# RMichelsen/VulkanHybridRenderer

Hardware: AMD Instinct MI355X
Metric: Mrays/s (unique rays) + ms/frame, Sponza 1080p RT shadows+AO+SVGF (higher is better)
Workload: dtype f32

## Files before the change

### vulkanhybridrenderer_amd/csrc/kernels_trace.hip

```cpp
#define VHR_TRACE_UNIT unit_trace
#include <cstring>

#include "trace_queue.hpp"
#include "svgf_temporal.hpp"

namespace vhr {

#ifndef VHR_REDO_INLINE
#define VHR_REDO_INLINE __attribute__((noinline))
#endif
#ifndef VHR_K1_WAVES_MIN
#define VHR_K1_WAVES_MIN 8
#endif
constexpr uint32_t kRedoPixel = 0x80000000u;

struct RaygenArgs {
    DeviceScene scene;
    vhr_per_frame_data pfd;
    vhr_trace_params tp;
    const void *normals;
    const float *depth;
    void *shadow_ao;
    void *reflections;
    uint32_t width, height;
// ... 20 lines not shown
    N = f3{ nid.x, nid.y, nid.z };
    origin = P + N * a.tp.normal_bias;
    Hit hit;

    float rnd1 = random01(rng);
    float rnd2 = random01(rng);
    shadow_payload = 1.0f;
    if (a.tp.shadow_enable) {
        const f3 cone_dir = normalize3(uniform_sample_cone(rnd1, rnd2, a.tp.cone_cos_max));
        const f3 dir = onb_transform(L, cone_dir);
        const bool occluded = traverse<true, STRIDE>(a.scene, origin, dir, a.tp.tmin, a.tp.tmax, stack, hit, overflow, ray_filter<FILTER>(a.scene, a.masks, a.masks.shadow));
        shadow_payload = occluded ? 0.0f : 1.0f;
    }
    ao_payload = 0.0f;
    for (uint32_t i = 0; i < a.tp.ao_spp; ++i) {
        rnd1 = random01(rng);
        rnd2 = random01(rng);
        const f3 rnd_dir = cosine_hemisphere(rnd1, rnd2);
        const f3 dir = onb_transform(N, rnd_dir);
        const bool occluded = traverse<true, STRIDE>(a.scene, origin, dir, a.tp.tmin, a.tp.ao_tmax, stack, hit, overflow, ray_filter<FILTER>(a.scene, a.masks, a.masks.ao));
        ao_payload += occluded ? 0.0f : 1.0f;
    }
    if (a.tp.ao_spp) ao_payload /= float(a.tp.ao_spp); else ao_payload = 1.0f;
}

template <int FILTER = kFilterNone>
__device__ VHR_REDO_INLINE float2 redo_pixel_visibility(const RaygenArgs *a, const uint32_t x, const uint32_t y) {
    int st[kTraceStack];
    uint32_t overflow = 0;
    f3 P, N, origin;
    float shadow_payload, ao_payload;
    pixel_visibility<1, FILTER>(*a, x, y, a->depth[size_t(y) * a->width + x], st, overflow, P, N, origin, shadow_payload, ao_payload);
    return float2{ shadow_payload, ao_payload };
}

template <int FILTER = kFilterNone>
__device__ __forceinline__ void raygen_pixel(const RaygenArgs &a, const uint32_t x, const uint32_t y, int *stack, uint32_t &overflow, bool &covered, bool &second_ray) {
    const uint32_t W = a.width;
    const float depth = a.depth[size_t(y) * W + x];
    if (depth == 0.0f) {
        store_rg16f(a.shadow_ao, W, x, y, 1.0f, 1.0f);
        if (a.reflections) store_rgba16f(a.reflections, W, x, y, 0.0f, 0.0f, 0.0f, 0.0f);
        return;
    }
    covered = true;
    f3 P, N, origin;
    float shadow_payload, ao_payload;
    pixel_visibility<kTraceBlock, FILTER>(a, x, y, depth, stack, overflow, P, N, origin, shadow_payload, ao_payload);
    store_rg16f(a.shadow_ao, W, x, y, shadow_payload, ao_payload);

    if (a.reflections) {
        f4 payload = f4{ 0.0f, 0.0f, 0.0f, 0.0f };
        if (a.tp.reflections) {
            const f3 cam = f3{ a.pfd.camera_view_inverse[12], a.pfd.camera_view_inverse[13], a.pfd.camera_view_inverse[14] };
            const f3 I = normalize3(P - cam);
            const float ni2 = 2.0f * dot3(N, I);
            const f3 rdir = I - N * ni2;
            payload = trace_reflection<kTraceBlock>(a.scene, a.pfd, a.tp, origin, rdir, stack, overflow, second_ray, ray_filter<FILTER>(a.scene, a.masks, a.masks.reflection));
        }
        store_rgba16f(a.reflections, W, x, y, payload.x, payload.y, payload.z, payload.w);
    }
}

template <int FILTER = kFilterNone>
__global__ __launch_bounds__(kTraceBlock) void raygen_kernel(const RaygenArgs a, const Stamps st) {
    vhr_stamp(st);
    __shared__ int s_stack[kTraceStack * kTraceBlock];
    int *stack = s_stack + threadIdx.x;
    uint32_t x, y;
    pixel_of_thread(x, y, a.row_begin);
    uint32_t overflow = 0;
    bool covered = false, second_ray = false;
    if (x < a.width && y < a.row_end) raygen_pixel<FILTER>(a, x, y, stack, overflow, covered, second_ray);
    if (a.stats) {
        const unsigned long long cov = __ballot(covered), ovf = __ballot(overflow != 0), sec = __ballot(second_ray);
        if ((threadIdx.x & 63u) == 0) {
            if (cov) atomicAdd(&a.stats->covered_pixels, (unsigned long long)__popcll(cov));
            if (ovf) atomicAdd(&a.stats->stack_overflows, (unsigned long long)__popcll(ovf));
            if (sec) atomicAdd(&a.stats->second_bounce_rays, (unsigned long long)__popcll(sec));
        }
    }
}

template <int WAVES, bool COMPACT, bool SPILL, bool STATS, bool FUSE = false, int FILTER = kFilterNone>
__global__ __launch_bounds__(kQueueBlock *WAVES) __attribute__((amdgpu_waves_per_eu(VHR_K1_WAVES_MIN, 8))) void raygen_queue_kernel(const RaygenArgs a, const uint32_t stack_levels, const uint32_t refill_threshold,
                                                                          const uint32_t block_tiles_x, const uint32_t early_exit, const uint32_t tile_rows, const uint32_t steal_threshold, const Stamps st) {
    vhr_stamp(st);
    RayStats *const stats = STATS ? a.stats : nullptr;
    extern __shared__ int s_dyn[];
    const unsigned long long t_start = stats ? __builtin_readcyclecounter() : 0ull;
    unsigned long long t_setup = 0, t_refill = 0, t_nodes = 0, t_leaves = 0, n_refills = 0;
    __shared__ uint32_t s_vis_all[WAVES][kQueueBlock];
    __shared__ float s_ray_all[WAVES][5][kQueueBlock];
    __shared__ uint8_t s_list_all[WAVES][kQueueBlock];
    __shared__ float4 s_cut_all[WAVES][kCutMax][2];
    const uint32_t lane = threadIdx.x & 63u, wave = uint32_t(__builtin_amdgcn_readfirstlane(int(threadIdx.x >> 6)));
    uint32_t (&s_vis)[kQueueBlock] = s_vis_all[wave];
    float (&s_ray)[5][kQueueBlock] = s_ray_all[wave];
    uint8_t (&s_list)[kQueueBlock] = s_list_all[wave];
    float4 (&s_cut)[kCutMax][2] = s_cut_all[wave];
    const unsigned long long t_cost0 = a.co.wave_cost ? __builtin_readcyclecounter() : 0ull;
    if constexpr (!STATS) {
        if (a.co.order_out && blockIdx.x == 0u) order_blocks_by_cost<WAVES>(a.co.cost_prev, a.co.order_blocks, a.co.order_out, reinterpret_cast<uint32_t *>(s_dyn));
    }
    int *stack = s_dyn + wave * (stack_levels + 3u) * kQueueBlock + lane;
    stack[0] = kStackSentinel;
    const uint32_t W = a.width, H = a.height;
    uint32_t x, y;
    const uint32_t block_tile = a.co.block_order ? a.co.block_order[blockIdx.x] : blockIdx.x;
    tile_pixel<WAVES>(block_tile, block_tiles_x, wave, lane, a.row_begin, tile_rows, x, y, a.col_begin);
    const bool in_range = x < a.col_end && y < a.row_end && (lane >> 3) < tile_rows;
    bool covered = false;
    float depth = 0.0f;
    if (in_range) {
        depth = a.depth[size_t(y) * W + x];
        covered = depth != 0.0f;
        if (!covered) store_rg16f(a.shadow_ao, W, x, y, 1.0f, 1.0f);
    }
    s_vis[lane] = 0;
    const uint32_t first_kind = a.tp.shadow_enable ? 0u : 1u;
    const uint32_t last_kind = a.tp.ao_spp;
    const bool ao_only = first_kind != 0u;
    const bool kind_bits = last_kind <= 30u;
    const f3 L = -f3{ a.pfd.directional_light.direction[0], a.pfd.directional_light.direction[1], a.pfd.directional_light.direction[2] };
    f3 omin = f3{ 3.0e38f, 3.0e38f, 3.0e38f }, omax = f3{ -3.0e38f, -3.0e38f, -3.0e38f };
    float ao_reach = 0.0f;
    if (covered) {
        const float u = (float(x) + 0.5f) / float(W);
        const float v = (float(y) + 0.5f) / float(H);
        const f3 P = get_world_space_position(a.pfd, depth, u, v);
        const uint2 nraw = reinterpret_cast<const uint2 *>(a.normals)[size_t(y) * W + x];
        const f3 N = f3{ half_bits_to_float(uint16_t(nraw.x & 0xffffu)), half_bits_to_float(uint16_t(nraw.x >> 16)), half_bits_to_float(uint16_t(nraw.y & 0xffffu)) };
        const f3 origin = P + N * a.tp.normal_bias;
        s_ray[0][lane] = origin.x; s_ray[1][lane] = origin.y; s_ray[2][lane] = origin.z;
        s_ray[3][lane] = __uint_as_float(nraw.x); s_ray[4][lane] = __uint_as_float(nraw.y);
        if (ao_only) ao_reach = a.tp.ao_tmax * onb_norm_bound(N);
        omin = origin; omax = origin;
    }
    const unsigned long long cov_mask = __ballot(covered);
    const uint32_t ncov = uint32_t(__popcll(cov_mask));
    if (covered) s_list[lane_rank(cov_mask)] = uint8_t(lane);
    wave_lds_sync();
    const uint32_t total = (a.scene.node_count == 0) ? 0u : ncov * (1u + last_kind - first_kind);
    uint32_t cut_n = 0;
    if (total) cut_n = build_tile_cut(a.scene, omin, omax, s_cut, lane, ao_only ? ao_reach : 3.0e38f, kCutMax, COMPACT ? int(sizeof(BvhNode16)) : int(sizeof(BvhNode48)),
                                      COMPACT ? f3{ a.scene.centre[0], a.scene.centre[1], a.scene.centre[2] } : f3{ 0.0f, 0.0f, 0.0f });
    const uint32_t n_cut_entries = cut_n;
    uint32_t emask = 0;
    if (stats) t_setup = __builtin_readcyclecounter() - t_start;

    f3 ro = f3{ 0, 0, 0 }, rd = f3{ 0, 0, 1 }, rinv = f3{ 0, 0, 0 }, noi = f3{ 0, 0, 0 }, ainv = f3{ 0, 0, 0 };
    float tmax = 0.0f;
    int cur = 0, sp = 0;
    int sbase = 0;
    uint32_t pix = 0, kind = 0;
    bool has = false;
    uint32_t next = 0;
    uint32_t overflow = 0;
    uint32_t n_nodes = 0, n_leaves = 0, n_tris = 0, n_wave_trips = 0, n_drain_trips = 0;
    uint32_t n_drain_le4 = 0, n_drain_le8 = 0, n_drain_le16 = 0;
    int spill[SPILL ? kSpillStack : 1];
    const float tmin = a.tp.tmin;
    float tmin_v = tmin;
    asm volatile("" : "+v"(tmin_v));
    for (;;) {
        const unsigned long long idle = __ballot(!has);
        const uint32_t n_idle = uint32_t(__popcll(idle));
        const unsigned long long t0 = stats ? __builtin_readcyclecounter() : 0ull;
        const bool queue_dry = next >= total;
        if (next < total && (n_idle >= refill_threshold || n_idle == 64u)) {
            __builtin_amdgcn_s_setprio(0);
            ++n_refills;
            const uint32_t r = next + lane_rank(idle);
            next += n_idle;
            if (!has && r < total) {
                uint32_t k = 0, rr = r;
                while (rr >= ncov) { rr -= ncov; ++k; }
                kind = last_kind - k;
                pix = s_list[rr];
                ro = f3{ s_ray[0][pix], s_ray[1][pix], s_ray[2][pix] };
                const uint32_t nxy = __float_as_uint(s_ray[3][pix]), nzw = __float_as_uint(s_ray[4][pix]);
                const uint32_t px = x - (lane & 7u) + (pix & 7u), py = y - (lane >> 3) + (pix >> 3);
                rd = ray_direction(a.tp, seed_thread((py * H + px) * a.pfd.frame_index), kind, L,
                                   f3{ half_bits_to_float(uint16_t(nxy & 0xffffu)), half_bits_to_float(uint16_t(nxy >> 16)), half_bits_to_float(uint16_t(nzw & 0xffffu)) });
                tmax = kind == 0 ? a.tp.tmax : a.tp.ao_tmax;
                f3 bo, bd;
                box_ray(a.scene, ro, rd, bo, bd);
                rinv = f3{ cull_reciprocal(bd.x), cull_reciprocal(bd.y), cull_reciprocal(bd.z) };
                const f3 oc = COMPACT ? f3{ bo.x - a.scene.centre[0], bo.y - a.scene.centre[1], bo.z - a.scene.centre[2] } : bo;
                noi = f3{ -(oc.x * rinv.x), -(oc.y * rinv.y), -(oc.z * rinv.z) };
                if (!COMPACT) ainv = f3{ fabsf(rinv.x), fabsf(rinv.y), fabsf(rinv.z) };
                sbase = 0;
                cut_to_stack(s_cut, cut_n, stack, stack_levels, rinv, noi, tmin_v, tmax, cur, sp, emask);
// ... 88 lines not shown
            const bool holder = has && cur < 0 && cur != kStackSentinel;
            uint32_t w = mine, hl = holder ? tot - mine : 0u, fr = holder ? 0u : tot - mine;
            for (int off = 32; off > 0; off >>= 1) { w += uint32_t(__shfl_xor(int(w), off)); hl += uint32_t(__shfl_xor(int(hl), off)); fr += uint32_t(__shfl_xor(int(fr), off)); }
            n_drain_le4 += w; n_drain_le8 += hl; n_drain_le16 += fr;
        }
#endif
        const unsigned long long t2 = stats ? __builtin_readcyclecounter() : 0ull;
        auto test_leaf = [&](const int code) {
            const uint32_t vv = ~uint32_t(code);
            const uint32_t first = vv >> 2, count = (vv & 3u) + 1u;
            ++n_leaves;
            const BvhTri *const leaf = a.scene.tris + first;
            for (uint32_t i = 0; i < count; ++i) {
                ++n_tris;
                const float4 ta = reinterpret_cast<const float4 *>(leaf + i)[0], tb = reinterpret_cast<const float4 *>(leaf + i)[1];
                const float tcx = reinterpret_cast<const float *>(leaf + i)[8];
                const f3 v0 = f3{ ta.x, ta.y, ta.z }, e1 = f3{ ta.w, tb.x, tb.y }, e2 = f3{ tb.z, tb.w, tcx };
                float ct, cu, cv;
                if (mt_candidate(ro, rd, v0, e1, e2, tmin, tmax, ct, cu, cv)) {
                    if (solution_consistent(ro, rd, v0, e1, e2, ct, cu, cv)) {
                        if constexpr (FILTER == kFilterAlpha) { if (gbuf_discarded(a.scene, first + i, cu, cv)) continue; }
                        if constexpr (FILTER == kFilterMask) {
                            if ((uint32_t(a.masks.prim_masks[leaf[i].prim]) & (kind == 0 ? a.masks.shadow : a.masks.ao)) == 0u) continue;
                            if (a.masks.alpha && gbuf_discarded(a.scene, first + i, cu, cv)) continue;
                        }
                        found = true;
                        break;
                    }
                    atomicOr(&s_vis[pix], kRedoPixel);
                }
            }
        };
        if (has && cur < 0 && cur != kStackSentinel) {
            test_leaf(cur);
            if (!found) {
                cur = stack[min(uint32_t(sp), stack_levels + 1u) * kQueueBlock];
                if (SPILL && __any(uint32_t(sp) > stack_levels)) {
                    if (uint32_t(sp) > stack_levels) cur = spill[(uint32_t(sp) - 1u - stack_levels) & uint32_t(kSpillStack - 1)];
                }
                --sp;
            }
        }
        if (has && !found && cur == kStackSentinel && emask) {
            const int e = __ffs(int(emask)) - 1;
            emask &= emask - 1u;
            cur = __float_as_int(s_cut[e][1].z);
            sp = 0;
            sbase = 0;
        }
        const bool finished = found || cur == kStackSentinel;
        if (has && finished) {
            has = false;
            if (kind_bits) { if (found) atomicOr(&s_vis[pix], 1u << kind); }
            else if (kind == 0) { if (found) atomicOr(&s_vis[pix], 1u); }
            else if (!found) atomicAdd(&s_vis[pix], 256u);
        }
        if (stats) {
            const unsigned long long t3 = __builtin_readcyclecounter();
            t_refill += t1 - t0; t_nodes += t2 - t1; t_leaves += t3 - t2;
            uint32_t tn = n_nodes - nodes_before, tt = n_tris - tris_before;
            for (int off = 32; off > 0; off >>= 1) { tn = max(tn, uint32_t(__shfl_xor(int(tn), off))); tt = max(tt, uint32_t(__shfl_xor(int(tt), off))); }
            n_wave_trips += tn + tt;
            if (next >= total) {
#ifndef VHR_K1_COUNT_TRIPS
                n_drain_trips += tn + tt;
#endif
                const uint32_t live = uint32_t(__popcll(__ballot(has)));
#ifndef VHR_K1_COUNT_IDLE
                if (live <= 4u) n_drain_le4 += tn + tt;
                if (live <= 8u) n_drain_le8 += tn + tt;
                if (live <= 16u) n_drain_le16 += tn + tt;
#endif
            }
        }
    }
    wave_lds_sync();
    float shadow_payload = 1.0f, ao_payload = 1.0f;
    uint32_t n_redo = 0;
    if (covered) {
        const uint32_t vis = s_vis[lane];
        shadow_payload = (vis & 1u) ? 0.0f : 1.0f;
        if (a.tp.ao_spp) ao_payload = float(a.scene.node_count == 0 ? a.tp.ao_spp : (kind_bits ? a.tp.ao_spp - uint32_t(__popc(vis >> 1)) : (vis >> 8))) / float(a.tp.ao_spp);
        if (vis & kRedoPixel) {
            static_assert(offsetof(RaygenArgs, scene) == 0, "the launch's arguments start with `a`");
            const float2 again = redo_pixel_visibility<FILTER>(reinterpret_cast<const RaygenArgs *>((const void *)__builtin_amdgcn_kernarg_segment_ptr()), x, y);
            shadow_payload = again.x; ao_payload = again.y;
            n_redo = 1;
        }
        store_rg16f(a.shadow_ao, W, x, y, shadow_payload, ao_payload);
    }
    if (a.co.wave_cost && lane == 0) a.co.wave_cost[block_tile * uint32_t(WAVES) + wave] = uint32_t(min(__builtin_readcyclecounter() - t_cost0, 0xffffffffull));
    if constexpr (FUSE) {
        if (a.fuse_temporal) {
            const TemporalArgs &t = a.temporal;
            if (in_range && x >= t.col_begin && x < t.limit_x && y >= t.row_begin && y < t.row_end && y < t.limit_y) {
                const uint2 nraw = reinterpret_cast<const uint2 *>(a.normals)[size_t(y) * W + x];
                const float2 cur = unpack_rg16f(pack_rg16f(shadow_payload, ao_payload));
                svgf_temporal_pixel(t, x, y, unpack_rgba16f(nraw), cur.x, cur.y);
            }
        }
    }
    if (stats) {
        const unsigned long long ovf = __ballot(overflow != 0);
        if (lane == 0) {
            if (cov_mask) atomicAdd(&stats->covered_pixels, (unsigned long long)__popcll(cov_mask));
            if (ovf) atomicAdd(&stats->stack_overflows, (unsigned long long)__popcll(ovf));
            atomicAdd(&stats->wave_iterations, (unsigned long long)n_wave_trips);
            atomicAdd(&stats->drain_iterations, (unsigned long long)n_drain_trips);
            atomicAdd(&stats->drain_le4, (unsigned long long)n_drain_le4);
            atomicAdd(&stats->drain_le8, (unsigned long long)n_drain_le8);
            atomicAdd(&stats->drain_le16, (unsigned long long)n_drain_le16);
            atomicAdd(&stats->cycles_total, __builtin_readcyclecounter() - t_start);
            atomicAdd(&stats->cycles_setup, t_setup);
            atomicAdd(&stats->cycles_refill, t_refill);
            atomicAdd(&stats->cycles_nodes, t_nodes);
            atomicAdd(&stats->cycles_leaves, t_leaves);
            atomicAdd(&stats->refills, n_refills);
            atomicAdd(&stats->waves, 1ull);
            atomicAdd(&stats->cut_entries, (unsigned long long)n_cut_entries);
        }
        const unsigned long long redo = __ballot(n_redo != 0);
        if (redo && lane == 0) atomicAdd(&stats->pending_rays, (unsigned long long)__popcll(redo));
        for (int off = 32; off > 0; off >>= 1) { n_nodes += uint32_t(__shfl_xor(int(n_nodes), off)); n_leaves += uint32_t(__shfl_xor(int(n_leaves), off)); n_tris += uint32_t(__shfl_xor(int(n_tris), off)); }
        if (lane == 0) {
            atomicAdd(&stats->node_visits, (unsigned long long)n_nodes);
            atomicAdd(&stats->leaf_visits, (unsigned long long)n_leaves);
            atomicAdd(&stats->triangle_tests, (unsigned long long)n_tris);
        }
    }
}

template <int STRIDE, int FILTER = kFilterNone>
__device__ __forceinline__ f4 reflection_payload(const RaygenArgs &a, const uint32_t x, const uint32_t y, int *stack, bool &second_ray) {
    const uint32_t W = a.width, H = a.height;
    f4 payload = f4{ 0.0f, 0.0f, 0.0f, 0.0f };
    const float depth = a.depth[size_t(y) * W + x];
    if (depth != 0.0f && a.tp.reflections) {
        const float u = (float(x) + 0.5f) / float(W), v = (float(y) + 0.5f) / float(H);
        const f3 P = get_world_space_position(a.pfd, depth, u, v);
        const f4 nid = load_rgba16f(a.normals, W, x, y);
        const f3 N = f3{ nid.x, nid.y, nid.z };
        const f3 origin = P + N * a.tp.normal_bias;
        const f3 cam = f3{ a.pfd.camera_view_inverse[12], a.pfd.camera_view_inverse[13], a.pfd.camera_view_inverse[14] };
        const f3 I = normalize3(P - cam);
        const float ni2 = 2.0f * dot3(N, I);
        const f3 rdir = I - N * ni2;
        uint32_t overflow = 0;
        payload = trace_reflection<STRIDE>(a.scene, a.pfd, a.tp, origin, rdir, stack, overflow, second_ray, ray_filter<FILTER>(a.scene, a.masks, a.masks.reflection));
    }
    return payload;
}
template <int FILTER = kFilterNone>
__device__ __forceinline__ void reflection_pixel(const RaygenArgs &a, const uint32_t x, const uint32_t y, int *stack, bool &second_ray) {
    const f4 payload = reflection_payload<kTraceBlock, FILTER>(a, x, y, stack, second_ray);
    store_rgba16f(a.reflections, a.width, x, y, payload.x, payload.y, payload.z, payload.w);
}

struct RedoReflection { f4 payload; uint32_t second; };
template <int FILTER = kFilterNone>
__device__ __attribute__((noinline)) RedoReflection redo_pixel_reflection(const RaygenArgs *a, const uint32_t x, const uint32_t y) {
    int st[kTraceStack];
    bool second_ray = false;
    const f4 payload = reflection_payload<1, FILTER>(*a, x, y, st, second_ray);
    return RedoReflection{ payload, second_ray ? 1u : 0u };
}

template <int FILTER = kFilterNone>
__global__ __launch_bounds__(kTraceBlock) void reflection_kernel(const RaygenArgs a, const Stamps st) {
    vhr_stamp(st);
    __shared__ int s_refl_stack[kTraceStack * kTraceBlock];
    int *stack = s_refl_stack + threadIdx.x;
    uint32_t x, y;
    pixel_of_thread(x, y, a.row_begin);
    bool second_ray = false;
    if (x < a.width && y < a.row_end) reflection_pixel<FILTER>(a, x, y, stack, second_ray);
    if (a.stats) {
        const unsigned long long sec = __ballot(second_ray);
        if ((threadIdx.x & 63u) == 0 && sec) atomicAdd(&a.stats->second_bounce_rays, (unsigned long long)__popcll(sec));
    }
}

__device__ __forceinline__ void mirror_ray_of_pixel(const RaygenArgs &a, f3 cam, uint32_t x, uint32_t y, float depth, f3 &origin, f3 &rdir) {
    const uint32_t W = a.width, H = a.height;
    const float u = (float(x) + 0.5f) / float(W), v = (float(y) + 0.5f) / float(H);
    const f3 P = get_world_space_position(a.pfd, depth, u, v);
    const f4 nid = load_rgba16f(a.normals, W, x, y);
    const f3 N = f3{ nid.x, nid.y, nid.z };
    origin = P + N * a.tp.normal_bias;
    const f3 I = normalize3(P - cam);
    const float ni2 = 2.0f * dot3(N, I);
    rdir = I - N * ni2;
}

template <bool SPILL, int BOUNCES, bool STATS = false, int FILTER = kFilterNone>
__global__ __launch_bounds__(kQueueBlock * 2) __attribute__((amdgpu_waves_per_eu(7, 7))) void reflection_queue_kernel(
    const RaygenArgs a, const uint32_t stack_levels, const uint32_t refill_threshold, const uint32_t tiles_x, const uint32_t tiles_total,
    const uint32_t early_exit, const Stamps st) {
    vhr_stamp(st);
    extern __shared__ int s_dyn[];
    constexpr int ROWS = BOUNCES > 1 ? 9 : 6;
    constexpr uint32_t SUBS = 1u;
    constexpr int RAYS = 64 * int(SUBS);
    __shared__ float s_ray_all[2][ROWS][RAYS];
    __shared__ uint8_t s_list_all[2][RAYS];
    __shared__ float4 s_cut_all[2][kCutMax][2];
    __shared__ uint32_t s_redo_all[2][RAYS / 32];
    const uint32_t lane = threadIdx.x & 63u, wave = uint32_t(__builtin_amdgcn_readfirstlane(int(threadIdx.x >> 6)));
    const unsigned long long t_cost0 = a.co.wave_cost ? __builtin_readcyclecounter() : 0ull;
    if (a.co.order_out && blockIdx.x == 0u) order_blocks_by_cost<2>(a.co.cost_prev, a.co.order_blocks, a.co.order_out, reinterpret_cast<uint32_t *>(s_dyn));
    const uint32_t block = a.co.block_order ? a.co.block_order[blockIdx.x] : blockIdx.x;
    const uint32_t tile = block * 2u + wave;
// ... 107 lines not shown
            static_assert(offsetof(RaygenArgs, scene) == 0, "the launch's arguments start with `a`");
            const RedoReflection again = redo_pixel_reflection<FILTER>(reinterpret_cast<const RaygenArgs *>((const void *)__builtin_amdgcn_kernarg_segment_ptr()), x, y);
            payload = again.payload;
            ++n_redo;
            if (BOUNCES > 1) redo_second += int(again.second) - int(tri != kNoHit);
        } else if (tri != kNoHit) {
            Hit h;
            h.t = 0.0f; h.u = s_ray[1][p]; h.v = s_ray[2][p]; h.tri_index = tri; h.flat = 0;
            if constexpr (BOUNCES > 1) {
                f4 second = f4{ 0.0f, 0.0f, 0.0f, 0.0f };
                const uint32_t tri2 = __float_as_uint(s_ray[6][p]);
                if (tri2 != kNoHit) {
                    Hit h2;
                    h2.t = 0.0f; h2.u = s_ray[7][p]; h2.v = s_ray[8][p]; h2.tri_index = tri2; h2.flat = 0;
                    second = shade_reflection_hit(a.scene, a.pfd, h2);
                }
                payload = shade_reflection_hit(a.scene, a.pfd, h, &second);
            } else {
                payload = shade_reflection_hit(a.scene, a.pfd, h);
            }
        }
        store_rgba16f(a.reflections, W, x, y, payload.x, payload.y, payload.z, payload.w);
    }
    if (a.stats) {
        for (int off = 32; off > 0; off >>= 1) { n_redo += uint32_t(__shfl_xor(int(n_redo), off)); redo_second += __shfl_xor(redo_second, off); }
        second_rays = uint32_t(int(second_rays) + redo_second);
        if (lane == 0) {
            if (overflow) atomicAdd(&a.stats->stack_overflows, 1ull);
            if (second_rays) atomicAdd(&a.stats->second_bounce_rays, (unsigned long long)second_rays);
            if (n_redo) atomicAdd(&(a.stats + 1)->pending_rays, (unsigned long long)n_redo);
        }
    }
    if constexpr (STATS) {
        RayStats *const rs = a.stats + 1;
        uint32_t n_nodes = wc.nodes, n_leaves = wc.leaves, n_tris = wc.triangles;
        for (int off = 32; off > 0; off >>= 1) { n_nodes += uint32_t(__shfl_xor(int(n_nodes), off)); n_leaves += uint32_t(__shfl_xor(int(n_leaves), off)); n_tris += uint32_t(__shfl_xor(int(n_tris), off)); }
        if (lane == 0) {
            atomicAdd(&rs->node_visits, (unsigned long long)n_nodes);
            atomicAdd(&rs->leaf_visits, (unsigned long long)n_leaves);
            atomicAdd(&rs->triangle_tests, (unsigned long long)n_tris);
            atomicAdd(&rs->wave_iterations, (unsigned long long)wc.wave_trips);
            atomicAdd(&rs->unique_rays, (unsigned long long)(ncov + second_rays));
            atomicAdd(&rs->covered_pixels, (unsigned long long)ncov);
            atomicAdd(&rs->second_bounce_rays, (unsigned long long)second_rays);
            atomicAdd(&rs->refills, (unsigned long long)wc.refills);
            atomicAdd(&rs->waves, 1ull);
            atomicAdd(&rs->cycles_total, __builtin_readcyclecounter() - t_walk0);
            atomicAdd(&rs->cycles_nodes, t_walk);
        }
    }
    if (a.co.wave_cost && lane == 0) a.co.wave_cost[tile] = uint32_t(min(__builtin_readcyclecounter() - t_cost0, 0xffffffffull));
}

static bool alpha_rays(const vhr_context *ctx) { return ctx->alpha_test_rays != 0 && ctx->scene_can_discard; }


static void issue_raygen(vhr_context *ctx, const RaygenArgs &a_in, const uint32_t width, const uint32_t height, const bool alpha = false, const int filter = kFilterNone) {
    RaygenArgs a = a_in;
    a.co = CostOrderArgs{};
    (void)height;
    ctx->time_begin(kKernelRaygen);
    if (alpha) ++ctx->alpha_launches;
    if (filter == kFilterMask) ++ctx->mask_launches;
    if (ctx->options[kOptRaygenVariant] == 0) {
        with_filter(filter, [&](auto al) { launch(ctx, raygen_kernel<decltype(al)::value>, dim3((width + 15) / 16, (a.row_end - a.row_begin + 15) / 16), dim3(kTraceBlock), 0, a); });
    } else {
        const uint32_t rows_traced = a.row_end - a.row_begin;
        uint32_t tile_rows = uint32_t(std::max(0, std::min(8, ctx->options[kOptRaygenTileRows])));
        if (tile_rows == 0u) {
            const uint64_t tiles8 = uint64_t((a.col_end - a.col_begin + 7) / 8) * ((rows_traced + 7) / 8), slots = uint64_t(ctx->cu_count) * 32u;
            tile_rows = tiles8 * 10u < slots * 7u ? 6u : 8u;
        }
        const uint32_t tiles_x = (a.col_end - a.col_begin + 7) / 8, tiles_y = (rows_traced + tile_rows - 1) / tile_rows;
        const int waves = ctx->options[kOptWavesPerBlock];
        const uint32_t wv = waves >= 4 ? 4u : (waves >= 2 ? 2u : 1u);
        const QueueLaunch q = queue_launch(ctx, kOptLdsStackLevels, kOptEarlyExit, wv);
        const bool compact = ctx->options[kOptCompactNodes] != 0 && ctx->nodes16_valid;
        const uint32_t n_blocks = ((tiles_x + wv - 1u) / wv) * tiles_y;
        {
            const uint32_t key = (tiles_x * 2654435761u) ^ (tiles_y * 40503u) ^ (wv << 28) ^ (tile_rows << 24) ^ (a.row_begin * 97u) ^ (a.col_begin * 193u);
            if (!a.stats && q.levels >= 5u) prepare_cost_order(ctx, ctx->cost_order_raygen, n_blocks, wv, key, a.co, { tiles_x, (tiles_x + wv - 1u) / wv, wv, 8u, tile_rows, a.col_begin, a.row_begin });
        }
        const uint32_t steal = uint32_t(std::max(0, std::min(63, ctx->options[kOptRaygenSteal])));
        auto go = [&](auto kernel) { launch(ctx, kernel, dim3(n_blocks), dim3(kQueueBlock * wv), q.lds_bytes, a, q.levels, q.threshold, (tiles_x + wv - 1u) / wv, q.early_exit, tile_rows, steal); };
        auto by_flags = [&](auto waves_c) {
            constexpr int WV = decltype(waves_c)::value;
            with_bool(q.spill, [&](auto sp) {
                constexpr bool SP = decltype(sp)::value;
                if (a.fuse_temporal && compact && !a.stats && filter == kFilterNone) {
                    go(raygen_queue_kernel<WV, true, SP, false, true>);
                    return;
                }
                with_bool(compact, [&](auto co) {
                    with_bool(a.stats != nullptr, [&](auto st) { with_filter(filter, [&](auto al) {
                        go(raygen_queue_kernel<WV, decltype(co)::value, SP, decltype(st)::value, false, decltype(al)::value>);
                    }); });
                });
            });
        };
        if (wv == 4u) by_flags(std::integral_constant<int, 4>{});
        else if (wv == 2u) by_flags(std::integral_constant<int, 2>{});
        else by_flags(std::integral_constant<int, 1>{});
    }
    ctx->time_end(kKernelRaygen);
}

struct DeferredRaygen { RaygenArgs a; uint32_t width, height; };
int flush_deferred_raygen(vhr_context *ctx, const TemporalArgs *fuse) {
    if (!ctx->deferred_raygen) return VHR_OK;
    DeferredRaygen d;
    std::memcpy(&d, ctx->deferred_raygen_blob.data(), sizeof(d));
    ctx->deferred_raygen = false;
    if (fuse) { d.a.fuse_temporal = 1u; d.a.temporal = *fuse; }
    PassDescription *const running = ctx->cur_pass;
    ctx->cur_pass = ctx->deferred_pass;
    issue_raygen(ctx, d.a, d.width, d.height);
    if (ctx->deferred_pass && ctx->deferred_pass->stamped_in_kernel) {
        ctx->pending_end = &ctx->d_stamps[ctx->deferred_pass->stamp_index].end;
        ctx->deferred_pass->timed = true;
    }
    ctx->cur_pass = running;
    ctx->deferred_pass = nullptr;
    if (hipGetLastError() != hipSuccess) return ctx->fail(VHR_ERROR_DEVICE, "raygen kernel launch failed");
    return VHR_OK;
}
bool deferred_raygen_matches(const vhr_context *ctx, const TemporalArgs &t) {
    if (!ctx->deferred_raygen) return false;
    DeferredRaygen d;
    std::memcpy(&d, ctx->deferred_raygen_blob.data(), sizeof(d));
    return t.raytraced == d.a.shadow_ao && static_cast<const void *>(t.normals) == d.a.normals && t.width == d.a.width && t.height == d.a.height &&
           t.col_begin == 0 && t.row_begin == 0 && t.limit_x == d.a.width && t.row_end >= d.a.height && t.limit_y >= d.a.height &&
           d.a.col_begin == 0 && d.a.row_begin == 0 && d.a.col_end == d.a.width && d.a.row_end == d.a.height;
}

int launch_raygen(vhr_context *ctx, const vhr_per_frame_data &pfd, uint32_t width, uint32_t height, const Image &normals,
                  const Image &depth, Image &shadow_ao, Image *reflections) {
    if (width != normals.width || height != normals.height || width != depth.width || height != depth.height ||
        width != shadow_ao.width || height != shadow_ao.height || (reflections && (reflections->width != width || reflections->height != height)))
        return ctx->fail(VHR_ERROR_INVALID_ARGUMENT, "TraceRays: launch size must equal the extent of the pass images");
    RaygenArgs a;
    a.fuse_temporal = 0u;
    a.temporal = TemporalArgs{};
    a.co = CostOrderArgs{};
    a.scene = ctx->device_scene();
    a.pfd = pfd;
    a.tp = ctx->trace_params;
    a.normals = normals.ptr;
    a.depth = static_cast<const float *>(depth.ptr);
    a.shadow_ao = shadow_ao.ptr;
    a.reflections = reflections ? reflections->ptr : nullptr;
    a.width = width;
    a.height = height;
    const uint32_t owned_begin = std::min(ctx->row_begin, height), owned_end = std::min(ctx->row_end, height);
    a.row_begin = owned_begin;
    a.row_end = owned_end;
    const uint32_t owned_col_begin = std::min(ctx->col_begin, width), owned_col_end = std::min(ctx->col_end, width);
    a.col_begin = owned_col_begin & ~15u;
    a.col_end = owned_col_end;
    a.stats = ctx->ray_stats_enabled ? ctx->d_ray_stats : nullptr;
    ctx->raytraced_pixels = 0;
    ctx->alpha_launches = 0;
    ctx->mask_launches = 0;
    if (a.row_end <= a.row_begin || a.col_end <= a.col_begin) return VHR_OK;
    if (ctx->options[kOptTraceOverlap]) {
        a.row_begin = owned_begin > ctx->overlap ? owned_begin - ctx->overlap : 0u;
        a.row_end = uint32_t(std::min<uint64_t>(height, uint64_t(owned_end) + ctx->overlap));
        a.col_begin = (owned_col_begin > ctx->overlap ? owned_col_begin - ctx->overlap : 0u) & ~15u;
// ... 93 lines not shown
```

### vulkanhybridrenderer_amd/csrc/trace_queue.hpp

```cpp
#pragma once

#include <algorithm>
#include <type_traits>

#include "trace_device.hpp"

namespace vhr {

typedef float f2v __attribute__((ext_vector_type(2)));

__device__ __forceinline__ float hw_min(float a, float b) { float r; asm("v_min_f32 %0, %1, %2" : "=v"(r) : "v"(a), "v"(b)); return r; }
__device__ __forceinline__ float hw_max(float a, float b) { float r; asm("v_max_f32 %0, %1, %2" : "=v"(r) : "v"(a), "v"(b)); return r; }
__device__ __forceinline__ float hw_min3(float a, float b, float c) { float r; asm("v_min3_f32 %0, %1, %2, %3" : "=v"(r) : "v"(a), "v"(b), "v"(c)); return r; }
__device__ __forceinline__ float hw_max3(float a, float b, float c) { float r; asm("v_max3_f32 %0, %1, %2, %3" : "=v"(r) : "v"(a), "v"(b), "v"(c)); return r; }

__device__ __forceinline__ unsigned long long cmp_le_mask(float a, float b) { unsigned long long m; asm("v_cmp_le_f32_e64 %0, %1, %2" : "=s"(m) : "v"(a), "v"(b)); return m; }
__device__ __forceinline__ unsigned long long cmp_gt_i32_mask_s(int uniform_a, int b) { unsigned long long m; asm("v_cmp_gt_i32_e64 %0, %1, %2" : "=s"(m) : "s"(uniform_a), "v"(b)); return m; }
__device__ __forceinline__ unsigned long long cmp_eq_i32_mask_s(int uniform_a, int b) { unsigned long long m; asm("v_cmp_eq_i32_e64 %0, %1, %2" : "=s"(m) : "s"(uniform_a), "v"(b)); return m; }
__device__ __forceinline__ int select_mask(int if_clear, int if_set, unsigned long long m) { int d; asm("v_cndmask_b32_e64 %0, %1, %2, %3" : "=v"(d) : "v"(if_clear), "v"(if_set), "s"(m)); return d; }

__device__ __forceinline__ bool box_test_pk(f2v bx, f2v by, f2v bz, f3 inv, f3 noi, float tmin, float tlimit, float &tnear) {
    const f2v tx = __builtin_elementwise_fma(bx, f2v{ inv.x, inv.x }, f2v{ noi.x, noi.x });
    const f2v ty = __builtin_elementwise_fma(by, f2v{ inv.y, inv.y }, f2v{ noi.y, noi.y });
    const f2v tz = __builtin_elementwise_fma(bz, f2v{ inv.z, inv.z }, f2v{ noi.z, noi.z });
// ... 441 lines not shown
            int *const row = stack + min(uint32_t(sp), stack_levels + 1u) * kQueueBlock;
            int top = row[0];
            row[kQueueBlock] = farc;
            if (__any(uint32_t(sp) >= stack_levels)) {
                if (SPILL && uint32_t(sp) > stack_levels) top = spill[(uint32_t(sp) - 1u - stack_levels) & uint32_t(kSpillStack - 1)];
                if (uint32_t(sp) >= stack_levels) {
                    if (SPILL && uint32_t(sp) - stack_levels < uint32_t(kSpillStack)) spill[uint32_t(sp) - stack_levels] = farc;
                    else overflow |= both ? 1u : 0u;
                }
            }
            cur = both ? nearc : (none ? top : (h0 ? links.x : links.y));
            sp += (both ? 1 : 0) - (none ? 1 : 0);
        }
        if (has && cur < 0 && cur != kStackSentinel) {
            const uint32_t vv = ~uint32_t(cur);
            const uint32_t first = vv >> 2, count = (vv & 3u) + 1u;
            bool done = false;
            if (STATS) ++wc->leaves;
            for (uint32_t i = 0; i < count; ++i) {
                const float4 *tp = reinterpret_cast<const float4 *>(sc.tris + first + i);
                const float4 ta = tp[0], tb = tp[1], tc = tp[2];
                float t, uu, ww;
                if (STATS) ++my_tris;
                const f3 v0 = f3{ ta.x, ta.y, ta.z }, e1 = f3{ ta.w, tb.x, tb.y }, e2 = f3{ tb.z, tb.w, tc.x };
                if (mt_candidate(ro, rd, v0, e1, e2, ray_tmin, ray_tmax, t, uu, ww)) {
                    if (!solution_consistent(ro, rd, v0, e1, e2, t, uu, ww)) {
                        if (DEFER) { flag(pix); continue; }
                        if (!mt_binary64(ro, rd, v0, e1, e2, ray_tmin, ray_tmax, t, uu, ww)) continue;
                    }
                    if constexpr (!std::is_same_v<Filter, NoFilter>) { if (filter(pix, first + i, uu, ww)) continue; }
                    const uint32_t flat = __float_as_uint(tc.w);
                    if (best_tri == kNoHit || t < tbest || (t == tbest && flat < best_flat)) {
                        tbest = t; best_tri = first + i; best_flat = flat; best_u = uu; best_v = ww;
                    }
                    if (any_hit) { done = true; break; }
                }
            }
            if (done) {
                cur = kStackSentinel;
                emask = 0;
            } else {
                cur = stack[min(uint32_t(sp), stack_levels + 1u) * kQueueBlock];
                if (SPILL && __any(uint32_t(sp) > stack_levels)) {
                    if (uint32_t(sp) > stack_levels) cur = spill[(uint32_t(sp) - 1u - stack_levels) & uint32_t(kSpillStack - 1)];
                }
                --sp;
            }
        }
        if (has && cur == kStackSentinel && emask) {
            const int e = __ffs(int(emask)) - 1;
            emask &= emask - 1u;
            cur = __float_as_int(cut[e][1].z);
            sp = 0;
        }
        if (has && cur == kStackSentinel) {
            has = false;
            if constexpr (PER_RAY) commit(pix, best_tri, best_u, best_v, tbest);
            else commit(pix, best_tri, best_u, best_v);
        }
        if (STATS) {
            wc->nodes += my_nodes; wc->triangles += my_tris;
            uint32_t tn = my_nodes, tt = my_tris;
            for (int off = 32; off > 0; off >>= 1) { tn = max(tn, uint32_t(__shfl_xor(int(tn), off))); tt = max(tt, uint32_t(__shfl_xor(int(tt), off))); }
            wc->wave_trips += tn + tt;
        }
    }
}

struct QueueLaunch {
    uint32_t levels, threshold, early_exit;
    size_t lds_bytes;
    bool spill;
};
static QueueLaunch queue_launch(const vhr_context *ctx, const int lds_levels_option, const int early_exit_option, const uint32_t waves_per_block) {
    QueueLaunch q;
    q.levels = std::max<uint32_t>(1u, std::min<uint32_t>(ctx->bvh_depth + 1u, uint32_t(std::max(1, ctx->options[lds_levels_option]))));
    q.threshold = uint32_t(std::max(1, std::min(64, ctx->options[kOptRefillThreshold])));
    q.early_exit = uint32_t(std::max(0, std::min(15, ctx->options[early_exit_option])));
    q.lds_bytes = size_t(q.levels + 3) * kQueueBlock * sizeof(int) * waves_per_block;
    q.spill = q.levels < ctx->bvh_depth + 1u;
    return q;
}

struct TileGrid {
    uint32_t tiles_x, tiles_total;
    dim3 grid, block;
};
static TileGrid tile_grid(const uint32_t columns, const uint32_t rows, const uint32_t tile_w) {
    TileGrid g;
    g.tiles_x = (columns + tile_w - 1u) / tile_w;
    g.tiles_total = g.tiles_x * ((rows + 7u) / 8u);
    g.grid = dim3((g.tiles_total + 1u) / 2u);
    g.block = dim3(kQueueBlock * 2);
    return g;
}

static int ray_stats_begin(vhr_context *ctx, const bool on, const uint32_t count = 1u) {
    if (on && hipMemsetAsync(ctx->d_ray_stats, 0, count * sizeof(RayStats), ctx->stream) != hipSuccess)
        return ctx->fail(VHR_ERROR_DEVICE, "hipMemsetAsync(ray stats) failed");
    return VHR_OK;
}
static int ray_stats_end(vhr_context *ctx, const bool on, const char *launch_failed, const uint32_t count = 1u) {
    if (hipGetLastError() != hipSuccess) return ctx->fail(VHR_ERROR_DEVICE, launch_failed);
    if (on && (hipMemcpyAsync(&ctx->h_ray_stats, ctx->d_ray_stats, sizeof(RayStats), hipMemcpyDeviceToHost, ctx->stream) != hipSuccess ||
               (count > 1u && hipMemcpyAsync(&ctx->h_refl_stats, ctx->d_ray_stats + 1, sizeof(RayStats), hipMemcpyDeviceToHost, ctx->stream) != hipSuccess)))
        return ctx->fail(VHR_ERROR_DEVICE, "hipMemcpyAsync(ray stats) failed");
    return VHR_OK;
}

template <typename F>
static void with_bool(const bool flag, F &&f) {
    if (flag) f(std::true_type{});
    else f(std::false_type{});
}
static int launch_filter(const bool mask_acts, const bool alpha) { return mask_acts ? kFilterMask : (alpha ? kFilterAlpha : kFilterNone); }
template <typename F>
static void with_filter(const int filter, F &&f) {
    if (filter == kFilterMask) f(std::integral_constant<int, kFilterMask>{});
    else if (filter == kFilterAlpha) f(std::integral_constant<int, kFilterAlpha>{});
    else f(std::integral_constant<int, kFilterNone>{});
}

static void prepare_cost_order(vhr_context *ctx, vhr_context::CostOrder &co, const uint32_t n_blocks, const uint32_t wv, const uint32_t key, CostOrderArgs &out,
                               const vhr_context::CostOrder::Shape &shape) {
    const int mode = ctx->options[kOptRaygenCostOrder];
    if (!mode) return;
    if (co.stream != ctx->stream) {
        if (co.capacity) (void)hipDeviceSynchronize();
        co.stream = ctx->stream;
        co.order_blocks[0] = co.order_blocks[1] = co.cost_blocks[0] = co.cost_blocks[1] = 0;
    }
    if (n_blocks < (mode >= 2 ? 2u : 2048u)) return;
    const uint32_t n_waves = n_blocks * wv;
    if (n_waves > co.capacity) {
        (void)hipDeviceSynchronize();
        for (int i = 0; i < 2; ++i) { (void)hipFree(co.cost[i]); (void)hipFree(co.order[i]); co.cost[i] = co.order[i] = nullptr; }
        co.capacity = 0;
        co.order_blocks[0] = co.order_blocks[1] = co.cost_blocks[0] = co.cost_blocks[1] = 0;
        bool ok = true;
        for (int i = 0; i < 2; ++i)
            ok = ok && hipMalloc(reinterpret_cast<void **>(&co.cost[i]), size_t(n_waves) * 4) == hipSuccess &&
                 hipMalloc(reinterpret_cast<void **>(&co.order[i]), size_t(n_waves) * 4) == hipSuccess;
        if (!ok) return;
        co.capacity = n_waves;
    }
    const uint32_t prev = co.slot, slot = prev ^ 1u;
    co.slot = slot;
    out.wave_cost = co.cost[slot];
    if (co.order_blocks[slot] == n_blocks && co.order_key[slot] == key) out.block_order = co.order[slot];
    if (co.cost_blocks[prev] == n_blocks && co.cost_key[prev] == key) {
        out.cost_prev = co.cost[prev]; out.order_out = co.order[prev]; out.order_blocks = n_blocks;
        co.order_blocks[prev] = n_blocks; co.order_key[prev] = key;
    } else {
        co.order_blocks[prev] = 0;
    }
    co.cost_blocks[slot] = n_blocks; co.cost_key[slot] = key;
    co.cost_waves[slot] = n_waves;
    co.shape[slot] = shape;
}

}
```

### vulkanhybridrenderer_amd/csrc/vhr_internal.hpp

```cpp
#pragma once

#include <hip/hip_runtime.h>
#include <hip/hip_ext.h>

#include <cstdint>
#include <map>
#include <string>
#include <unordered_map>
#include <vector>

#include "vhr_amd.h"

namespace vhr {

struct BvhNode {
    float box0[6];
    float box1[6];
    int32_t child0, child1;
    int32_t pad[2];
};
static_assert(sizeof(BvhNode) == 64, "BvhNode");

struct BvhNode16 {
    uint16_t c[6];
// ... 199 lines not shown
    bool begin_stamped = false, end_on_last_dispatch = false;
    bool stamped_in_kernel = false;
    int stamp_index = -1;
    double ema_ms = 0.0, last_ms = 0.0;
};

struct TemporalArgs {
    const uint2 *normals, *motion, *prev_normals, *history;
    const uint32_t *raytraced, *moments_in;
    uint2 *integrated_out;
    uint32_t *moments_out;
    uint32_t width, height;
    uint32_t limit_x, limit_y;
    uint32_t row_begin, row_end;
    uint32_t col_begin;
    float display_w, display_h;
};
struct AtrousArgs {
    const uint2 *normals, *in;
    uint2 *out;
    uint2 *out2;
    uint2 *normals_out;
    uint32_t width, height, limit_x, limit_y, row_begin, row_end;
    uint32_t col_begin;
    int32_t step;
    float display_w, display_h;
};
struct SvgfCmd {
    enum Kind { Temporal, Atrous, Copy } kind;
    TemporalArgs t;
    AtrousArgs a;
    const char *copy_src; char *copy_dst; size_t copy_bytes;
    size_t copy_pitch, copy_row_bytes; uint32_t copy_rows;
    const void *src_base; void *dst_base;
};

struct RayQueryCounters { uint32_t redo_count, overflows; unsigned long long hits; };
struct RayQueryScratch { hipStream_t stream; RayQueryCounters *counters; uint32_t *list; uint64_t capacity; };
struct PointQueryCounters { unsigned long long found, evaluations; uint32_t overflows, pad; };
struct PointQueryScratch { hipStream_t stream; PointQueryCounters *counters; };

struct RayStats {
    unsigned long long unique_rays, covered_pixels, stack_overflows, node_visits, leaf_visits, triangle_tests, wave_iterations, second_bounce_rays;
    unsigned long long cycles_total, cycles_setup, cycles_refill, cycles_nodes, cycles_leaves, refills, waves, drain_iterations;
    unsigned long long cut_entries;
    unsigned long long drain_le4, drain_le8, drain_le16;
    unsigned long long pending_rays, pending_retraces;
};

#define VHR_OPTION_TABLE(X)                                                                                                             \
                            \
    X(kOptRaygenVariant, "raygen_variant", 1, 0, 1)              \
    X(kOptReflectionVariant, "reflection_variant", 1, 0, 1)            \
    X(kOptRaytracedVariant, "raytraced_variant", 1, 0, 1)        \
    X(kOptAtrousVariant, "atrous_variant", 1, 0, 1)              \
                                                                                                                 \
    X(kOptRefillThreshold, "refill_threshold", 16, 1, 64)               \
    X(kOptLdsStackLevels, "lds_stack_levels", 8, 1, 32)          \
    X(kOptReflectionLdsStackLevels, "reflection_lds_stack_levels", 10, 1, 32)  \
    X(kOptWavesPerBlock, "raygen_waves_per_block", 2, 1, 4)         \
    X(kOptCompactNodes, "compact_nodes", 1, 0, 1)                         \
    X(kOptEarlyExit, "raygen_early_exit", 6, 0, 15)              \
    X(kOptReflectionEarlyExit, "reflection_early_exit", 8, 0, 15)  \
    X(kOptRaygenTileRows, "raygen_tile_rows", 0, 0, 8)           \
    X(kOptRaygenCostOrder, "raygen_cost_order", 1, 0, 2)         \
    X(kOptRaygenSteal, "raygen_steal", 8, 0, 63)                 \
                                                                                                                \
    X(kOptAtrousSmallTiles, "atrous_small_tiles", -1, -1, 1)     \
                                                                                                              \
    X(kOptFuseBlits, "fuse_blits", 1, 0, 1)                                        \
    X(kOptSvgfElideUnread, "svgf_elide_unread", 0, 0, 1)         \
    X(kOptSvgfAsyncUnread, "svgf_async_unread", 1, 0, 2)          \
    X(kOptReflectionAsync, "reflection_async", 1, 0, 2)           \
    X(kOptFuseTemporal, "fuse_temporal", 0, 0, 1)                             \
    X(kOptFramesInFlight, "frames_in_flight", 1, 1, 3)                                                      \
                                                                                   \
    X(kOptTraceOverlap, "trace_overlap", 0, 0, 1)                \
    X(kOptShrinkOverlap, "strip_shrink_overlap", 0, 0, 1)            \
                                                                                                                   \
    X(kOptPassTimestamps, "pass_timestamps", 1, 0, 3)            \
    X(kOptKernelTimingStride, "kernel_timing_stride", 1, 1, 1000000)    \
                          \
    X(kOptRayqueryVariant, "variant_rayquery", 1, 0, 1)          \
    X(kOptForwardRasterVariant, "variant_standin_forward_raster", 1, 0, 1)

enum Option {
#define X(e, n, d, lo, hi) e,
    VHR_OPTION_TABLE(X)
#undef X
    kOptCount
};
struct OptionInfo { const char *name; int def, lo, hi; };
inline constexpr OptionInfo kOptionInfo[kOptCount] = {
#define X(e, n, d, lo, hi) { n, d, lo, hi },
    VHR_OPTION_TABLE(X)
#undef X
};

enum KernelKind { kKernelRaygen = 0, kKernelTemporal = 1, kKernelAtrous = 2, kKernelCopy = 3, kKernelReflection = 4, kKernelSsao = 5, kKernelSsaoBlur = 6, kKernelSsr = 7, kKernelAtrousAsync = 8, kKernelRayQuery = 9,
                  kKernelRayqueryForward = 10, kKernelForwardRaster = 11, kKernelKinds = 12,
                  kKernelRefit = 12 };
struct KernelTimer {
    std::vector<hipEvent_t> events;
    size_t used = 0;
    uint64_t seen = 0;
    double total_ms = 0.0;
    uint64_t launches = 0;
};

}

struct vhr_raytracing_execution_context {
    vhr_context *ctx;
    vhr::PassDescription *pass;
    uint32_t resource_idx;
};
struct vhr_compute_execution_context {
    vhr_context *ctx;
    vhr::PassDescription *pass;
    uint32_t resource_idx;
};

struct vhr_context {
    int device = 0;
    bool host_only = false;
    uint32_t width = 0, height = 0;
    hipStream_t stream = nullptr;
    bool own_stream = false;
    std::string error;

    static constexpr uint32_t kMaxGlobalResources = 2048;
    std::vector<vhr::Image> storage_images;
    struct Texture { void *texels; uint32_t w, h; int32_t format; vhr_sampler_info sampler; };
    std::vector<Texture> textures;
    vhr::DeviceTexture *d_textures = nullptr;
    bool textures_dirty = false;
    vhr_per_frame_data per_frame[3] = {};
    uint32_t last_resource_idx = 0;
    vhr_trace_params trace_params = {};

    vhr_vertex *d_vertices = nullptr;
    uint32_t *d_indices = nullptr;
    vhr_primitive *d_primitives = nullptr;
    float *d_normal_matrices = nullptr;
    vhr::BvhNode *d_nodes = nullptr;
    vhr::BvhNode16 *d_nodes16 = nullptr;
    vhr::BvhNodeCH *d_nodes_ch = nullptr;
    vhr::BvhNode48 *d_nodes48 = nullptr;
    uint64_t bvh_fingerprint = 0;
    uint64_t bvh_tree_fingerprint = 0;
    bool bvh_fingerprint_valid = false;
    int alpha_test_rays = 0;
    bool scene_can_discard = false;
    uint32_t alpha_launches = 0;
    std::vector<uint8_t> h_prim_masks;
    uint8_t *d_prim_masks = nullptr;
    uint64_t mask_present[4] = { 0, 0, 0, 1ull << 63 };
    uint64_t masks_not_ff = 0;
    int shadow_ray_mask = 255, ao_ray_mask = 255, reflection_ray_mask = 255;
    uint32_t mask_launches = 0;
    uint32_t rq_mask_ran = 0;
    bool ray_mask_acts(uint32_t m) const {
        for (uint32_t v = 0; v < 256u; ++v)
            if (((mask_present[v >> 6] >> (v & 63u)) & 1u) && (v & m) == 0u) return true;
        return false;
    }
    int object_motion_vectors = 0;
// ... 188 lines not shown
```

Measured before the change: 13480.

## Let raygen queue blocks loop over several tiles with wave-level ticket stealing

Adds a persistent-style mode in which a share of raygen queue blocks each own several consecutive tiles. Waves within such a block draw tickets from an LDS counter to pick up the next tile-wave as soon as they finish. The aim is to smooth wave-level load imbalance and cut block launch and setup overhead. Kernel arguments are packed into a single struct, and the kernarg pointer is re-read inside the loop to limit register pressure. It also adds a __syncthreads at start, per-iteration LDS atomics, and extra loop control, and it reduces the number of blocks in flight.

```diff
diff --git a/vulkanhybridrenderer_amd/csrc/kernels_trace.hip b/vulkanhybridrenderer_amd/csrc/kernels_trace.hip
--- a/vulkanhybridrenderer_amd/csrc/kernels_trace.hip
+++ b/vulkanhybridrenderer_amd/csrc/kernels_trace.hip
@@ -126,14 +126,16 @@
     }
 }
 
+struct RaygenQueueArgs {
+    RaygenArgs a;
+    uint32_t stack_levels, refill_threshold, block_tiles_x, early_exit, tile_rows, steal_threshold;
+    uint32_t block_tiles, looping_blocks;
+};
 template <int WAVES, bool COMPACT, bool SPILL, bool STATS, bool FUSE = false, int FILTER = kFilterNone>
-__global__ __launch_bounds__(kQueueBlock *WAVES) __attribute__((amdgpu_waves_per_eu(VHR_K1_WAVES_MIN, 8))) void raygen_queue_kernel(const RaygenArgs a, const uint32_t stack_levels, const uint32_t refill_threshold,
-                                                                          const uint32_t block_tiles_x, const uint32_t early_exit, const uint32_t tile_rows, const uint32_t steal_threshold, const Stamps st) {
+__global__ __launch_bounds__(kQueueBlock *WAVES) __attribute__((amdgpu_waves_per_eu(VHR_K1_WAVES_MIN, 8))) void raygen_queue_kernel(const RaygenQueueArgs args, const Stamps st) {
     vhr_stamp(st);
-    RayStats *const stats = STATS ? a.stats : nullptr;
+    RayStats *const stats = STATS ? args.a.stats : nullptr;
     extern __shared__ int s_dyn[];
-    const unsigned long long t_start = stats ? __builtin_readcyclecounter() : 0ull;
-    unsigned long long t_setup = 0, t_refill = 0, t_nodes = 0, t_leaves = 0, n_refills = 0;
     __shared__ uint32_t s_vis_all[WAVES][kQueueBlock];
     __shared__ float s_ray_all[WAVES][5][kQueueBlock];
     __shared__ uint8_t s_list_all[WAVES][kQueueBlock];
@@ -143,16 +145,35 @@
     float (&s_ray)[5][kQueueBlock] = s_ray_all[wave];
     uint8_t (&s_list)[kQueueBlock] = s_list_all[wave];
     float4 (&s_cut)[kCutMax][2] = s_cut_all[wave];
-    const unsigned long long t_cost0 = a.co.wave_cost ? __builtin_readcyclecounter() : 0ull;
+    __shared__ uint32_t s_ticket;
+    const bool looping = blockIdx.x < args.looping_blocks;
+    if (looping && threadIdx.x == 0u) s_ticket = uint32_t(WAVES);
+    unsigned long long t_cost0 = args.a.co.wave_cost ? __builtin_readcyclecounter() : 0ull;
+    bool synced = false;
     if constexpr (!STATS) {
-        if (a.co.order_out && blockIdx.x == 0u) order_blocks_by_cost<WAVES>(a.co.cost_prev, a.co.order_blocks, a.co.order_out, reinterpret_cast<uint32_t *>(s_dyn));
-    }
-    int *stack = s_dyn + wave * (stack_levels + 3u) * kQueueBlock + lane;
+        if (args.a.co.order_out && blockIdx.x == 0u) { order_blocks_by_cost<WAVES>(args.a.co.cost_prev, args.a.co.order_blocks, args.a.co.order_out, reinterpret_cast<uint32_t *>(s_dyn)); synced = true; }
+    }
+    if (looping && !synced) __syncthreads();
+    int *stack = s_dyn + wave * (args.stack_levels + 3u) * kQueueBlock + lane;
+    for (uint32_t ticket = wave;;) {
+    static_assert(offsetof(RaygenQueueArgs, a) == 0 && offsetof(RaygenArgs, scene) == 0, "the launch's arguments start with `args`, and those with the scene");
+    auto kernarg = __builtin_amdgcn_kernarg_segment_ptr();
+    asm volatile("" : "+s"(kernarg));
+    const RaygenQueueArgs &q = *reinterpret_cast<const RaygenQueueArgs *>((const void *)kernarg);
+    const RaygenArgs &a = q.a;
+    const uint32_t stack_levels = q.stack_levels, refill_threshold = q.refill_threshold, block_tiles_x = q.block_tiles_x, early_exit = q.early_exit, tile_rows = q.tile_rows,
+                   steal_threshold = q.steal_threshold;
+    const uint32_t positions = blockIdx.x < q.looping_blocks ? q.block_tiles : 1u;
+    const uint32_t first_position = blockIdx.x < q.looping_blocks ? blockIdx.x * q.block_tiles : q.looping_blocks * q.block_tiles + (blockIdx.x - q.looping_blocks);
+    const uint32_t position = first_position + ticket / uint32_t(WAVES), tile_wave = ticket % uint32_t(WAVES);
+    if (position >= gridDim.x + q.looping_blocks * (q.block_tiles - 1u)) break;
+    const uint32_t W = a.width, H = a.height;
+    const unsigned long long t_start = stats ? __builtin_readcyclecounter() : 0ull;
+    unsigned long long t_setup = 0, t_refill = 0, t_nodes = 0, t_leaves = 0, n_refills = 0;
     stack[0] = kStackSentinel;
-    const uint32_t W = a.width, H = a.height;
     uint32_t x, y;
-    const uint32_t block_tile = a.co.block_order ? a.co.block_order[blockIdx.x] : blockIdx.x;
-    tile_pixel<WAVES>(block_tile, block_tiles_x, wave, lane, a.row_begin, tile_rows, x, y, a.col_begin);
+    const uint32_t block_tile = a.co.block_order ? a.co.block_order[position] : position;
+    tile_pixel<WAVES>(block_tile, block_tiles_x, tile_wave, lane, a.row_begin, tile_rows, x, y, a.col_begin);
     const bool in_range = x < a.col_end && y < a.row_end && (lane >> 3) < tile_rows;
     bool covered = false;
     float depth = 0.0f;
@@ -407,14 +428,13 @@
         shadow_payload = (vis & 1u) ? 0.0f : 1.0f;
         if (a.tp.ao_spp) ao_payload = float(a.scene.node_count == 0 ? a.tp.ao_spp : (kind_bits ? a.tp.ao_spp - uint32_t(__popc(vis >> 1)) : (vis >> 8))) / float(a.tp.ao_spp);
         if (vis & kRedoPixel) {
-            static_assert(offsetof(RaygenArgs, scene) == 0, "the launch's arguments start with `a`");
-            const float2 again = redo_pixel_visibility<FILTER>(reinterpret_cast<const RaygenArgs *>((const void *)__builtin_amdgcn_kernarg_segment_ptr()), x, y);
+            const float2 again = redo_pixel_visibility<FILTER>(&a, x, y);
             shadow_payload = again.x; ao_payload = again.y;
             n_redo = 1;
         }
         store_rg16f(a.shadow_ao, W, x, y, shadow_payload, ao_payload);
     }
-    if (a.co.wave_cost && lane == 0) a.co.wave_cost[block_tile * uint32_t(WAVES) + wave] = uint32_t(min(__builtin_readcyclecounter() - t_cost0, 0xffffffffull));
+    if (a.co.wave_cost && lane == 0) a.co.wave_cost[block_tile * uint32_t(WAVES) + tile_wave] = uint32_t(min(__builtin_readcyclecounter() - t_cost0, 0xffffffffull));
     if constexpr (FUSE) {
         if (a.fuse_temporal) {
             const TemporalArgs &t = a.temporal;
@@ -452,6 +472,14 @@
             atomicAdd(&stats->leaf_visits, (unsigned long long)n_leaves);
             atomicAdd(&stats->triangle_tests, (unsigned long long)n_tris);
         }
+    }
+    if (positions == 1u) break;
+    uint32_t drawn = 0;
+    if (lane == 0u) drawn = atomicAdd(&s_ticket, 1u);
+    ticket = uint32_t(__builtin_amdgcn_readfirstlane(int(drawn)));
+    if (ticket >= positions * uint32_t(WAVES)) break;
+    wave_lds_sync();
+    if (a.co.wave_cost) t_cost0 = __builtin_readcyclecounter();
     }
 }
 
@@ -725,7 +753,10 @@
             if (!a.stats && q.levels >= 5u) prepare_cost_order(ctx, ctx->cost_order_raygen, n_blocks, wv, key, a.co, { tiles_x, (tiles_x + wv - 1u) / wv, wv, 8u, tile_rows, a.col_begin, a.row_begin });
         }
         const uint32_t steal = uint32_t(std::max(0, std::min(63, ctx->options[kOptRaygenSteal])));
-        auto go = [&](auto kernel) { launch(ctx, kernel, dim3(n_blocks), dim3(kQueueBlock * wv), q.lds_bytes, a, q.levels, q.threshold, (tiles_x + wv - 1u) / wv, q.early_exit, tile_rows, steal); };
+        const BlockTiles bt = block_tiles(ctx, n_blocks);
+        auto go = [&](auto kernel) {
+            launch(ctx, kernel, dim3(bt.grid), dim3(kQueueBlock * wv), q.lds_bytes, RaygenQueueArgs{ a, q.levels, q.threshold, (tiles_x + wv - 1u) / wv, q.early_exit, tile_rows, steal, bt.tiles, bt.looping });
+        };
         auto by_flags = [&](auto waves_c) {
             constexpr int WV = decltype(waves_c)::value;
             with_bool(q.spill, [&](auto sp) {
diff --git a/vulkanhybridrenderer_amd/csrc/trace_queue.hpp b/vulkanhybridrenderer_amd/csrc/trace_queue.hpp
--- a/vulkanhybridrenderer_amd/csrc/trace_queue.hpp
+++ b/vulkanhybridrenderer_amd/csrc/trace_queue.hpp
@@ -547,6 +547,15 @@
     return q;
 }
 
+struct BlockTiles { uint32_t grid, tiles, looping; };
+static BlockTiles block_tiles(const vhr_context *ctx, const uint32_t n_blocks) {
+    const uint32_t tiles = uint32_t(std::max(1, std::min(4, ctx->options[kOptRaygenBlockTiles])));
+    const uint32_t quarters = uint32_t(std::max(1, std::min(4, ctx->options[kOptRaygenBlockTilesShare])));
+    if (tiles == 1u || n_blocks < (ctx->options[kOptRaygenCostOrder] >= 2 ? 2u : 2048u)) return BlockTiles{ n_blocks, 1u, 0u };
+    const uint32_t looping = uint32_t(uint64_t(n_blocks) * quarters / 4u) / tiles;
+    return BlockTiles{ looping + (n_blocks - looping * tiles), tiles, looping };
+}
+
 struct TileGrid {
     uint32_t tiles_x, tiles_total;
     dim3 grid, block;
diff --git a/vulkanhybridrenderer_amd/csrc/vhr_internal.hpp b/vulkanhybridrenderer_amd/csrc/vhr_internal.hpp
--- a/vulkanhybridrenderer_amd/csrc/vhr_internal.hpp
+++ b/vulkanhybridrenderer_amd/csrc/vhr_internal.hpp
@@ -305,7 +305,10 @@
     X(kOptKernelTimingStride, "kernel_timing_stride", 1, 1, 1000000)    \
                           \
     X(kOptRayqueryVariant, "variant_rayquery", 1, 0, 1)          \
-    X(kOptForwardRasterVariant, "variant_standin_forward_raster", 1, 0, 1)
+    X(kOptForwardRasterVariant, "variant_standin_forward_raster", 1, 0, 1)    \
+     \
+    X(kOptRaygenBlockTiles, "raygen_block_tiles", 2, 1, 4)       \
+    X(kOptRaygenBlockTilesShare, "raygen_block_tiles_share", 2, 1, 4)
 
 enum Option {
 #define X(e, n, d, lo, hi) e,
```

Result: no change. 13350 (-0.9%).
